# axoloto/CudaCam

Measured on AMD Instinct MI355X. Metric: frames/sec, 1920x1080 grayscale Canny (5-stage, Mode R, device-resident), higher is better.
Workload: dtype u8

## Files before the change

### cudacam_amd/api.py

```python
import ctypes as C
import enum
import os
import sys

import numpy as np

_HERE = os.path.dirname(os.path.abspath(__file__))
LIB_PATH = os.environ.get("HIPCANNY_LIB") or os.path.join(_HERE, "libhipcanny.so")


class CannyStage(enum.IntEnum):
    MONO = 0
    GAUSSIAN = 1
    GRADIENT = 2
    NMS = 3
    THRESH = 4
    HYSTER = 5


CANNY_STAGES = {
    CannyStage.MONO: "1/6 Mono Conversion",
    CannyStage.GAUSSIAN: "2/6 Gaussian Noise Removal",
    CannyStage.GRADIENT: "3/6 Gradient Computation",
    CannyStage.NMS: "4/6 Non Maximum Suppression",
# ... 4 lines not shown
MODE_R, MODE_O = 0, 1
OPT_NMS_SATURATE = 1
OPT_PIPELINE = 2
OPT_PER_CHANNEL = 3
OPT_FRONT_SPLIT = 4
OPT_L2_GRADIENT = 5
OPT_DEBUG_TAPS = 6
OPT_FRONT_HALF = 7
OPT_FRONT_DENSE = 8
OPT_COPY_STREAMS = 9
OPT_PIPELINE_SLOTS = 10
OPT_FRONT_WPB = 11
OPT_FRONT_MX = 12
OPT_APERTURE = 13
OPT_TEST_HYST_LATE_GRID, OPT_TEST_HYST_LOOP, OPT_TEST_HYST_DIAG, OPT_TEST_HYST_GEOM, OPT_TEST_DENSE_ENTER, OPT_TEST_DENSE_LEAVE = 100, 101, 102, 103, 104, 105
TAP_BLUR, TAP_THRESH = 1, 2
SCHEDULE_FIELDS = ("launches", "lists", "loop", "hist_grid", "longest", "overflows", "tiles", "tile_rows", "waves", "panels", "frames")

ABI_SYMBOLS = [
    "hc_create", "hc_destroy", "hc_set_thresholds", "hc_get_thresholds", "hc_upload", "hc_run", "hc_run_device",
    "hc_hysteresis_device", "hc_download", "hc_sync", "hc_set_stream", "hc_enable_profiling", "hc_stage_time_ms", "hc_profile_get",
    "hc_device_ptrs", "hc_last_hysteresis_info", "hc_hysteresis_stats", "hc_set_tuning", "hc_set_option", "hc_selftest", "hc_last_error", "hc_version",
    "hc_host_alloc", "hc_host_free", "hc_profile_get_front", "hc_debug_tap", "hc_use_own_stream", "hc_profile_get_intervals", "hc_last_run_info", "hc_pipeline_depth", "hc_pipeline_slots_in_use", "hc_front_waves_per_workgroup",
    "hc_profile_get_front_each", "hc_hysteresis_totals", "hc_last_hysteresis_schedule", "hc_download_begin", "hc_download_end", "hc_run_gradients_device",
]

_lib = None
_lib_legacy = None
LEGACY_LIB_PATH = os.path.join(_HERE, "libhipcanny_legacy.so")


class HipCannyError(RuntimeError):
    pass


def preload_hip_runtime():
    import importlib.util
    spec = importlib.util.find_spec("torch")
    if spec is None or not spec.origin:
# ... 40 lines not shown
    L.hc_device_ptrs.argtypes = [vp, C.POINTER(vp), C.POINTER(vp), C.POINTER(sz), C.POINTER(sz), C.POINTER(sz), C.POINTER(sz)]
    L.hc_last_hysteresis_info.argtypes = [vp, C.POINTER(i), C.POINTER(i)]
    L.hc_hysteresis_stats.argtypes = [vp, C.POINTER(C.c_uint), i]
    L.hc_set_tuning.argtypes = [vp, i, i]
    L.hc_set_option.argtypes = [vp, i, i]
    L.hc_selftest.argtypes = [i]
    L.hc_debug_tap.argtypes = [vp, i, vp, sz, sz, i]
    L.hc_last_run_info.argtypes = [vp, C.POINTER(i), C.POINTER(i), C.POINTER(i)]
    L.hc_pipeline_depth.argtypes = [vp, i]
    L.hc_pipeline_slots_in_use.argtypes = [vp]
    L.hc_front_waves_per_workgroup.argtypes = [vp]
    L.hc_profile_get_intervals.argtypes = [vp, C.POINTER(C.c_float), i, C.POINTER(i)]
    L.hc_profile_get_front_each.argtypes = [vp, C.POINTER(C.c_float), i, C.POINTER(i)]
    L.hc_hysteresis_totals.argtypes = [vp, C.POINTER(C.c_ulonglong), i]
    L.hc_last_hysteresis_schedule.argtypes = [vp, C.POINTER(i), i]
    L.hc_host_alloc.restype = vp
    L.hc_host_alloc.argtypes = [sz]
    L.hc_host_free.restype = None
    L.hc_host_free.argtypes = [vp]
    L.hc_last_error.restype = C.c_char_p
    L.hc_version.restype = C.c_char_p
    for name in ABI_SYMBOLS:
        getattr(L, name)
    if legacy:
        _lib_legacy = L
    else:
        _lib = L
    return L


# ... 81 lines not shown
    def profile_front_each(self, cap=4096):
        buf = (C.c_float * cap)()
        n = C.c_int()
        _ck(self.lib.hc_profile_get_front_each(self.handle, buf, cap, C.byref(n)))
        return [buf[k] for k in range(min(cap, n.value))]

    def hysteresis_totals(self, reset=False):
        t = (C.c_ulonglong * 4)()
        _ck(self.lib.hc_hysteresis_totals(self.handle, t, int(bool(reset))))
        return tuple(int(v) for v in t)

    def hysteresis_schedule(self):
        v = (C.c_int * len(SCHEDULE_FIELDS))()
        _ck(self.lib.hc_last_hysteresis_schedule(self.handle, v, len(SCHEDULE_FIELDS)))
        return dict(zip(SCHEDULE_FIELDS, (int(x) for x in v)))

    def profile_get_front(self):
        sums = (C.c_double * 2)()
        n = C.c_long()
        _ck(self.lib.hc_profile_get_front(self.handle, sums, C.byref(n)))
        return [sums[0], sums[1]], n.value

    def upload(self, frames):
        a = np.ascontiguousarray(frames, dtype=np.uint8)
        if a.ndim == (2 if self.c == 1 else 3):
            a = a[None]
        exp = (self.h, self.w) if self.c == 1 else (self.h, self.w, 3)
        if a.shape[1:] != exp:
            raise HipCannyError(f"Cannot load image to GPU, specs different since initialization: {a.shape[1:]} vs {exp}")
        row = self.w * self.c
# ... 237 lines not shown
```

### cudacam_amd/csrc/canny_common.h

```cpp
#pragma once
#include <hip/hip_runtime.h>
#include "canny_params.h"

namespace hc {

hipError_t launch_selftest(u32 *d_result, hipStream_t s);
hipError_t check_gauss_coeffs(const float gk[25]);
hipError_t launch_front_o(const FrontParams &p, hipStream_t s);
hipError_t launch_front_o_ext(const FrontExtParams &p, hipStream_t s);
#ifdef HC_LEGACY_FRONT
hipError_t launch_front(const FrontParams &p, hipStream_t s);
hipError_t launch_blur(const FrontParams &p, hipStream_t s);
hipError_t launch_nms(const FrontParams &p, hipStream_t s);
size_t front_lds_bytes();
#endif
hipError_t launch_front8(const FrontParams &p, hipStream_t s);
hipError_t launch_front8o(const FrontParams &p, hipStream_t s);
hipError_t launch_front_mx(const FrontParams &p, hipStream_t s);
hipError_t launch_hyst(const HystParams &p, hipStream_t s);
hipError_t launch_hyst_loop(const HystParams &p, int rounds, u32 *bar, hipStream_t s);
hipError_t launch_pack(const PackParams &p, hipStream_t s);
hipError_t launch_copy_rows(void *dst, size_t dpitch, size_t dfs, const void *src, size_t spitch, size_t sfs, size_t row_bytes, int rows, int n, hipStream_t s);

hipError_t launch_gray(const uint8_t *bgr, size_t bpitch, size_t bfs, uint8_t *mono, size_t mpitch, size_t mfs, int W, int H, int n, hipStream_t s);
hipError_t launch_gauss(const uint8_t *mono, size_t mpitch, size_t mfs, uint8_t *blur, size_t bpitch, size_t bfs, int W, int H, int n, hipStream_t s);
hipError_t launch_sobel(const uint8_t *blur, size_t bpitch, size_t bfs, int16_t *sx, int16_t *sy, size_t spitch_elems, size_t sfs_elems, int W, int H, int n, hipStream_t s);
hipError_t launch_graddisp(const int16_t *sx, const int16_t *sy, size_t spitch_elems, size_t sfs_elems, uint8_t *out, size_t opitch, size_t ofs, int W, int H, int n, hipStream_t s);
hipError_t launch_nms(const int16_t *sx, const int16_t *sy, size_t spitch_elems, size_t sfs_elems, uint8_t *out, size_t opitch, size_t ofs, int W, int H, int n, int saturate, hipStream_t s);
hipError_t launch_thresh(const uint8_t *nms, size_t npitch, size_t nfs, uint8_t *out, size_t opitch, size_t ofs, int W, int H, int n, int low, int high, hipStream_t s);

}
```

### cudacam_amd/csrc/canny_kernels.hip

```cpp
#include "canny_device.h"
#include <cstdio>
#include <cstdlib>
#include <cstring>
#include <type_traits>

namespace hc {

hipError_t check_gauss_coeffs(const float gk[25])
{
  return memcmp(gk, GKC.v, sizeof(GKC.v)) == 0 ? hipSuccess : hipErrorInvalidValue;
}

__global__ void k_selftest(u32 *res)
{
  const u32 lane = threadIdx.x & 63;
  u32 bad = 0;
  bad |= (from_lane_below(lane + 100) != (lane ? lane + 99 : 0)) ? 1u : 0u;
  bad |= (from_lane_above(lane + 100) != (lane < 63 ? lane + 101 : 0)) ? 2u : 0u;
  const u32 x = 0x44332211u + lane;
  bad |= (unpack_lo(x) != ((x & 0xFF) | (((x >> 8) & 0xFF) << 16))) ? 4u : 0u;
  bad |= (unpack_hi(x) != (((x >> 16) & 0xFF) | ((x >> 24) << 16))) ? 8u : 0u;
  bad |= (pair_shift(0xAAAA1111u + lane, 0x2222BBBBu) != (((0xAAAA1111u + lane) << 16) | 0x2222u)) ? 16u : 0u;
  const u32 p0 = 0x00050003u, p1 = 0x00090007u;
  bad |= (__builtin_amdgcn_perm(p1, p0, 0x06040200u) != 0x09070503u) ? 32u : 0u;
// ... 305 lines not shown
  uint8_t *d = dst + (size_t)f * dfs + (size_t)row * dpitch + x;
  if (x + 16u <= row_bytes) *reinterpret_cast<u32x4_any *>(d) = *reinterpret_cast<const u32x4_any *>(q);
  else
    for (unsigned k = 0; x + k < row_bytes; ++k) d[k] = q[k];
}

hipError_t launch_copy_rows(void *dst, size_t dpitch, size_t dfs, const void *src, size_t spitch, size_t sfs, size_t row_bytes, int rows, int n, hipStream_t s)
{
  if (row_bytes == 0 || rows <= 0 || n <= 0) return hipSuccess;
  if (row_bytes > 0x7FFFFFFFull || rows > 65535 || n > 65535) return hipErrorInvalidValue;
  const dim3 grid((unsigned)((row_bytes + 4095) / 4096), (unsigned)rows, (unsigned)n), block(256);
  hipLaunchKernelGGL(k_copy_rows, grid, block, 0, s, (uint8_t *)dst, dpitch, dfs, (const uint8_t *)src, spitch, sfs, (unsigned)row_bytes, rows);
  return hipGetLastError();
}

hipError_t launch_pack(const PackParams &p, hipStream_t s)
{
  const long long total = (long long)p.nframes * p.H * ((p.W + 255) / 256);
  hipLaunchKernelGGL(k_pack, dim3((unsigned)((total + 3) / 4)), dim3(256), 0, s, p);
  return hipGetLastError();
}

template <int NW>
struct RowBits {
  u32 w[NW];
};

template <int NW>
static __device__ __forceinline__ RowBits<NW> row_load(const u32 *plane_row, int lane, int RD)
{
// ... 691 lines not shown
```

### cudacam_amd/csrc/hipcanny.hip

```cpp
#include "../../include/hipcanny.h"
#include "canny_common.h"
#include "host_plan.h"

#include <algorithm>
#include <cstdio>
#include <cstdlib>
#include <cstring>
#include <mutex>
#include <string>
#include <vector>

using namespace hc;

namespace {
constexpr int MAX_DEVICES = 64;
hipStream_t g_h2d[MAX_DEVICES] = { nullptr }, g_d2h[MAX_DEVICES] = { nullptr };
std::mutex g_copy_streams_mutex;
thread_local std::string g_err;
int fail(int code, const std::string &msg)
{
  g_err = msg;
  return code;
}
#define HIPCK(expr)                                                                                   \
  do {                                                                                                \
    hipError_t e_ = (expr);                                                                           \
    if (e_ != hipSuccess) return fail(HC_E_HIP, std::string(#expr) + ": " + hipGetErrorString(e_));  \
  } while (0)

struct Slot {
  bool complete = false;
  u32 *d_sbits = nullptr, *d_cbits = nullptr;
  u32 *d_wl_list = nullptr;
  size_t wl_cap = 0;
  u32 *d_flags = nullptr, *h_flags = nullptr;
  hipEvent_t ev_front = nullptr, ev_done = nullptr;
  bool pending = false;
  HystParams ph{};
  HystPlan plan;
  void *copy_dst = nullptr;
  size_t copy_pitch = 0, copy_fs = 0;
  int n = 0;
  bool prov = false;
  hipStream_t stream = nullptr;
  hipStream_t s_hyst = nullptr;
  uintptr_t out0 = 0, out1 = 0;
  unsigned long long seq = 0;
};

struct ProfRing {
// ... 94 lines not shown
  size_t in_pitch = 0, in_fs = 0, mono_pitch = 0, mono_fs = 0, out_pitch = 0, out_fs = 0;
  uint8_t *d_blur = nullptr, *d_nms = nullptr;
  int16_t *d_sx = nullptr, *d_sy = nullptr;
  uint8_t *d_dump = nullptr;
  size_t dump_region = 0;
  uint8_t *d_bplane = nullptr;
  size_t bplane_fs = 0, bplane_frames = 0;
  Slot slot[NSLOT];
  int nslot_use = 2;
  int cur = 0;
  bool pipeline = false;
  unsigned long long run_seq = 0;
  ChainWatch watch;
  struct { hipEvent_t f[8] = {}, d[8] = {}; unsigned long long seq[8] = {}; } ring;
  HystHistory hist;
  ProfRing prof;
  struct {
    uint8_t *host = nullptr; size_t row = 0, fs = 0; int n = 0;
    bool stale = false;
  } dl;
  bool copy_streams = false;
  hipEvent_t ev_up = nullptr, ev_ready = nullptr, ev_ready2 = nullptr, ev_down = nullptr;
  struct {
    u32 *s = nullptr, *c = nullptr;
    uint8_t *blur = nullptr;
    int frames = 0;
    bool blur_split = false, blur_valid = false;
  } dbg;
  struct {
    int front_waves = 4;
// ... 29 lines not shown
  return HC_OK;
}

int alloc_slot_parts(hc_ctx *c, Slot &s)
{
  const size_t out_frames = (size_t)c->max_batch * (c->per_channel ? 3 : 1);
  const size_t plane_bytes = sizeof(u32) * (size_t)c->RD * c->H * out_frames;
  HIPCK(hipMalloc((void **)&s.d_sbits, plane_bytes));
  HIPCK(hipMalloc((void **)&s.d_cbits, plane_bytes));
  HIPCK(hipMemsetAsync(s.d_sbits, 0, plane_bytes, c->stream));
  HIPCK(hipMemsetAsync(s.d_cbits, 0, plane_bytes, c->stream));
  HIPCK(hipStreamSynchronize(c->stream));
  s.wl_cap = slot_wl_cap(out_frames, c->H, c->RD);
  HIPCK(hipMalloc((void **)&s.d_wl_list, sizeof(u32) * 2 * s.wl_cap));
  HIPCK(hipMalloc((void **)&s.d_flags, sizeof(u32) * run_flag_words(s.wl_cap)));
  HIPCK(hipHostMalloc((void **)&s.h_flags, sizeof(u32) * (FLAG_WORDS + WL_COUNT_WORDS), hipHostMallocDefault));
  {
    int least = 0, greatest = 0;
    (void)hipDeviceGetStreamPriorityRange(&least, &greatest);
    HIPCK(hipStreamCreateWithPriority(&s.s_hyst, hipStreamNonBlocking, greatest));
  }
  HIPCK(hipEventCreateWithFlags(&s.ev_front, hipEventDisableTiming));
  HIPCK(hipEventCreateWithFlags(&s.ev_done, hipEventDisableTiming));
  return HC_OK;
}

void free_slot(Slot &s)
{
  for (void *q : { (void *)s.d_sbits, (void *)s.d_cbits, (void *)s.d_wl_list, (void *)s.d_flags }) (void)hipFree(q);
  if (s.h_flags) (void)hipHostFree(s.h_flags);
  if (s.ev_front) (void)hipEventDestroy(s.ev_front);
// ... 1 lines not shown
  if (s.s_hyst) (void)hipStreamDestroy(s.s_hyst);
  s = Slot{};
}

int alloc_slot(hc_ctx *c, Slot &s)
{
  if (s.complete) return HC_OK;
  const int rc = alloc_slot_parts(c, s);
  if (rc != HC_OK) {
    const std::string why = g_err;
    free_slot(s);
    return fail(rc, why);
  }
  s.complete = true;
  return HC_OK;
}

#ifdef HC_LEGACY_FRONT
int ensure_blur_plane(hc_ctx *c)
{
  const size_t frames = (size_t)c->max_batch * (c->per_channel ? 3 : 1);
  if (c->d_bplane && c->bplane_frames == frames) return HC_OK;
  if (c->d_bplane) { (void)hipFree(c->d_bplane); c->d_bplane = nullptr; }
  c->bplane_fs = (size_t)c->nstrips * c->H * 256;
  HIPCK(hipMalloc((void **)&c->d_bplane, c->bplane_fs * frames));
  c->bplane_frames = frames;
  return HC_OK;
}
#endif

// ... 48 lines not shown
  if (c->ring.seq[b] != i || c->ring.seq[a] != i - 1 || i < 2) return;
  float front_ms = 0.0f, lead_ms = 0.0f;
  if (hipEventElapsedTime(&front_ms, c->ring.f[a], c->ring.f[b]) != hipSuccess || hipEventElapsedTime(&lead_ms, c->ring.d[a], c->ring.f[b]) != hipSuccess) {
    (void)hipGetLastError();
    return;
  }
  c->watch.update(i, c->nslot_use, front_ms, lead_ms);
}

int finish_slot(hc_ctx *c, Slot &s)
{
  if (!s.pending) return HC_OK;
  s.pending = false;
  s.out0 = s.out1 = 0;
  hipStream_t st = s.stream;
  HIPCK(hipEventSynchronize(s.ev_done));
  watch_chain(c, s);
  const HystPlan &p = s.plan;
  const int K = p.K;
  int work = 0;
  for (int k = 0; k < K; ++k) work += s.h_flags[k] != 0;
  work = std::min(K, work + 1);
  std::memcpy(c->last.stats, s.h_flags + MAX_HYST_LAUNCHES, sizeof(c->last.stats));
  c->last.continued = 0;
  c->last.totals[0] += 1;
  c->last.totals[3] += (unsigned long long)K;
  u32 wl_counts[MAX_HYST_LAUNCHES + 1];
  std::memcpy(wl_counts, s.h_flags + FLAG_WORDS, sizeof(wl_counts));
  {
    int *d = c->last.sched;
    d[HC_SCHED_LAUNCHES] = K; d[HC_SCHED_LISTS] = p.mixed ? 2 : p.lists0; d[HC_SCHED_LOOP] = p.loop ? 1 : 0;
// ... 3 lines not shown
      const u32 len = wl_counts[k];
      d[HC_SCHED_LONGEST] = std::max(d[HC_SCHED_LONGEST], (int)std::min<u32>(len, 0x7FFFFFFFu));
      if (p.hist_grid(k) <= 0) continue;
      d[HC_SCHED_HIST_GRID] = d[HC_SCHED_HIST_GRID] ? std::min(d[HC_SCHED_HIST_GRID], p.hist_grid(k)) : p.hist_grid(k);
      if (len > (u32)p.hist_grid(k)) d[HC_SCHED_OVERFLOWS] += 1;
    }
    d[HC_SCHED_TILES] = (int)std::min<size_t>(p.wl_stride, 0x7FFFFFFF); d[HC_SCHED_TILE_ROWS] = p.tile_rows; d[HC_SCHED_WAVES] = p.waves;
    d[HC_SCHED_PANELS] = p.npanels; d[HC_SCHED_FRAMES] = s.ph.nframes;
  }
  const bool converged = s.h_flags[K - 1] == 0;
  if (!converged) {
    c->last.continued = 1;
    c->last.totals[1] += 1;
    if (c->dl.host) c->dl.stale = true;
    for (int round = 0; round < 1000000; ++round) {
      HIPCK(hipMemsetAsync(s.d_flags, 0, sizeof(u32) * run_flag_words(p.wl_stride), st));
      HystParams hp = s.ph;
      hp.late_grid = p.test_grid;
      hp.first_pass = 0;
      hp.stats = nullptr;
      for (int k = 0; k < K; ++k) {
        hp.iter = k;
        hp.lists = p.lists[k];
        HIPCK(launch_hyst(hp, st));
      }
      HIPCK(hipMemcpyAsync(s.h_flags, s.d_flags, sizeof(u32) * (FLAG_WORDS + WL_COUNT_WORDS), hipMemcpyDeviceToHost, st));
      HIPCK(hipStreamSynchronize(st));
      for (int k = 0; k < K; ++k) work += s.h_flags[k] != 0;
      if (s.h_flags[K - 1] == 0) break;
    }
  }
  c->last.totals[2] += (unsigned long long)work;
  c->hist.finished(p, work, wl_counts);
  if (converged) return HC_OK;
  if (s.copy_dst)
    if (int rc = copy_frames_d2d(c, st, s.copy_dst, s.copy_pitch, s.copy_fs, s.ph.out, s.ph.out_pitch, s.ph.out_frame_stride, (size_t)c->W, s.n)) return rc;
  HIPCK(hipStreamSynchronize(st));
  return HC_OK;
}

int finish_all(hc_ctx *c)
// ... 15 lines not shown
  hp.tile_rows = p.tile_rows; hp.waves = p.waves; hp.nrtiles = p.nrtiles; hp.npanels = p.npanels;
  hp.out = out; hp.out_pitch = out_pitch; hp.out_frame_stride = out_fs; hp.W = c->W;
  hp.wl_stride = p.wl_stride;
  hp.wl_count = s.d_flags + FLAG_WORDS;
  hp.wl_reason = s.d_flags + FLAG_WORDS + WL_COUNT_WORDS;
  hp.wl_list = s.d_wl_list;
  hp.first_pass = 1;
  hp.prov = s.prov ? 1 : 0;
  if (p.clear) HIPCK(hipMemsetAsync(s.d_flags, 0, sizeof(u32) * run_flag_words(p.wl_stride), st));
  if (p.loop) HIPCK(launch_hyst_loop(hp, p.K, s.d_flags + FLAG_WORDS + WL_COUNT_WORDS - 2, st));
  for (int k = p.loop ? p.K : 0; k < p.K; ++k) {
    hp.iter = k; hp.lists = p.lists[k]; hp.late_grid = p.late_grid[k];
    hp.stats = c->hopt.diag ? s.d_flags + MAX_HYST_LAUNCHES + 3 * k : nullptr;
    HIPCK(launch_hyst(hp, st));
  }
  HIPCK(hipMemcpyAsync(s.h_flags, s.d_flags, sizeof(u32) * (FLAG_WORDS + WL_COUNT_WORDS), hipMemcpyDeviceToHost, st));
  s.pending = true;
  s.ph = hp;
  s.n = n;
  s.stream = st;
  s.copy_dst = nullptr;
  return HC_OK;
}

int rotate_slots(hc_ctx *c, bool piped, int n_out, Slot **slot)
{
  if (piped) {
    const int use = pipeline_slots(c->watch.pipe_slots, c->watch.big_slots, n_out, c->W, c->H);
    if (use != c->nslot_use) {
      if (int rc = finish_all(c)) return rc;
      c->nslot_use = use;
      c->cur = 0;
    }
  }
  Slot &s = c->slot[piped ? c->cur : 0];
  *slot = &s;
  if (!piped) { s.seq = 0; return finish_all(c); }
  if (int rc = alloc_slot(c, s)) return rc;
  if (int rc = finish_slot(c, s)) return rc;
  s.seq = ++c->run_seq;
  return HC_OK;
}

int finish_overlapping(hc_ctx *c, uintptr_t o0, uintptr_t o1, bool *with_previous)
{
  *with_previous = false;
  for (int k = 1; k < c->nslot_use; ++k) {
    Slot &o = c->slot[(c->cur + k) % c->nslot_use];
    if (!(o.out0 < o1 && o0 < o.out1)) continue;
    if (k == c->nslot_use - 1) *with_previous = true;
    if (int rc = finish_slot(c, o)) return rc;
  }
  return HC_OK;
}

int run_impl(hc_ctx *c, const uint8_t *in, size_t in_pitch, size_t in_fs, uint8_t *out, size_t out_pitch, size_t out_fs, int n, int stage,
// ... 3 lines not shown
    return fail(HC_E_ARG, "mode O (cv::Canny) produces the final edge map only (cv::Canny has no intermediate outputs)");
  if (c->mode == HC_MODE_O && c->per_channel) return fail(HC_E_ARG, "HC_OPT_PER_CHANNEL applies to mode R contexts");
  if (c->per_channel && stage != HC_STAGE_HYSTER) return fail(HC_E_ARG, "per-channel mode only produces the final edge maps (HC_STAGE_HYSTER)");
  const int W = c->W, H = c->H;
  const int n_out = c->per_channel ? 3 * n : n;
  const bool piped = c->pipeline && stage == HC_STAGE_HYSTER;
  Slot *slot = nullptr;
  if (int rc = rotate_slots(c, piped, n_out, &slot)) return rc;
  Slot &s = *slot;
  FrontIn fi{ c->mode, c->C, W, H, c->RD, c->nstrips, c->per_channel, stage, n };
  fi.in = View{ (uintptr_t)in, in_pitch, in_fs }; fi.out = View{ (uintptr_t)out, out_pitch, out_fs }; fi.in_dy = (uintptr_t)in_dy;
  fi.own_in = View{ 0, c->in_pitch, c->in_fs }; fi.own_mono = View{ 0, c->mono_pitch, c->mono_fs }; fi.own_out = View{ 0, c->out_pitch, c->out_fs };
  fi.o = c->opt; fi.dump_region = c->dump_region; fi.piped = piped; fi.nslot_use = c->nslot_use; fi.front_one = c->watch.front_one; fi.wl_cap = s.wl_cap;
  const bool out_internal = out_view_staged(fi.out);
  uint8_t *dst = out_internal ? c->d_out : out;
  if (piped) {
    const uintptr_t o0 = (uintptr_t)dst, o1 = o0 + (size_t)n_out * (out_internal ? c->out_fs : out_fs);
    if (int rc = finish_overlapping(c, o0, o1, &fi.out_overlap)) return rc;
    s.out0 = o0; s.out1 = o1;
  }
  const FrontPlan P = plan_front(fi);
  c->last.in_staged = P.in_staged ? 1 : 0;
  c->last.out_staged = P.out_staged ? 1 : 0;
  c->last.front_form = P.form;
  if (P.error) return fail(HC_E_ARG, P.error);
  hipStream_t sf = c->stream, sh = piped ? s.s_hyst : c->stream;
  const size_t dp = P.dst.pitch, dfs = P.dst.fs;
  const uint8_t *src = P.in_staged ? c->d_in : in;
  if (P.in_staged)
    if (int rc = copy_frames_d2d(c, sf, c->d_in, c->in_pitch, c->in_fs, in, in_pitch, in_fs, (size_t)W * c->C, n)) return rc;
  ProfRing &prof = c->prof;
  HIPCK(prof.begin_run(sf));
  const uint8_t *mono = src;
  if (P.gray) {
    uint8_t *grey = stage == HC_STAGE_MONO ? dst : c->d_mono;
    HIPCK(launch_gray(src, P.src.pitch, P.src.fs, grey, stage == HC_STAGE_MONO ? dp : c->mono_pitch, stage == HC_STAGE_MONO ? dfs : c->mono_fs, W, H, n, sf));
    if (stage != HC_STAGE_MONO) mono = c->d_mono;
    HIPCK(prof.mark(sf, B_MONO, ProfRing::K_STAGE0));
  } else if (stage == HC_STAGE_MONO) {
    if (int rc = copy_frames_d2d(c, sf, dst, dp, dfs, src, P.src.pitch, P.src.fs, (size_t)W, n)) return rc;
    HIPCK(prof.mark(sf, B_MONO, ProfRing::K_STAGE0));
  }
  const size_t mp = P.mono.pitch, mfs = P.mono.fs;

  if (stage == HC_STAGE_HYSTER) {
    FrontParams fp = P.fp;
    fp.in = mono; fp.sbits = s.d_sbits; fp.cbits = s.d_cbits;
    s.prov = P.prov;
    if (P.prov) fp.prov_out = dst;
    if (c->opt.debug_taps) {
      if (int rc = ensure_debug_buffers(c)) return rc;
      if (P.form != 1) fp.dbg_blur = c->dbg.blur;
    }
    if (P.zeroed_words) {
      const size_t R = c->dump_region;
      fp.zero_words = s.d_flags;
      fp.dump = c->d_dump; fp.dump_c = c->d_dump + (fp.half ? R : 2048); fp.dump_p = c->d_dump + (fp.half ? 2 * R : 4096);
      fp.zeros = c->d_dump + (fp.half ? 3 * R : 16384);
    }
    if (P.waves) c->last.front_waves = P.waves;
    switch (P.form) {
    case 6: case 7: {
      FrontExtParams ep{};
      ep.f = fp;
      ep.gradients = in_dy ? 1 : 0;
      ep.channels = c->C;
      ep.dy = in_dy;
      HIPCK(launch_front_o_ext(ep, sf));
      break;
    }
    case 3: HIPCK(launch_front8o(fp, sf)); break;
    case -1: HIPCK(launch_front_o(fp, sf)); break;
    case 5: HIPCK(launch_front_mx(fp, sf)); break;
    case 2: case 4: HIPCK(launch_front8(fp, sf)); break;
#ifdef HC_LEGACY_FRONT
    case 1:
      if (int rc = ensure_blur_plane(c)) return rc;
      fp.blur = c->d_bplane; fp.blur_frame_stride = c->bplane_fs;
      HIPCK(launch_blur(fp, sf));
      HIPCK(prof.mark(sf, P.mask_a, ProfRing::K_FRONT_A));
      HIPCK(launch_nms(fp, sf));
      break;
    case 0: HIPCK(launch_front(fp, sf)); break;
#endif
    default: return fail(HC_E_ARG, "internal: front kernel form");
    }
    HIPCK(prof.mark(sf, P.mask, ProfRing::K_FRONT_B));
    if (c->opt.debug_taps) {
      const size_t bytes = sizeof(u32) * (size_t)c->RD * H * (size_t)n_out;
      HIPCK(hipMemcpyAsync(c->dbg.s, s.d_sbits, bytes, hipMemcpyDeviceToDevice, sf));
      HIPCK(hipMemcpyAsync(c->dbg.c, s.d_cbits, bytes, hipMemcpyDeviceToDevice, sf));
      c->dbg.frames = n_out;
      c->dbg.blur_split = P.form == 1;
      c->dbg.blur_valid = c->mode == HC_MODE_R;
    }
    if (piped) {
      HIPCK(hipEventRecord(s.ev_front, sf));
      const int k = (int)(s.seq & 7);
      if (!c->ring.f[k]) { HIPCK(hipEventCreate(&c->ring.f[k])); HIPCK(hipEventCreate(&c->ring.d[k])); }
      HIPCK(hipEventRecord(c->ring.f[k], sf));
      c->ring.seq[k] = 0;
      HIPCK(hipStreamWaitEvent(sh, s.ev_front, 0));
    }
    if (int rc = queue_hyst_expand(c, s, sh, dst, dp, dfs, n_out, piped, P.zeroed_words)) return rc;
  } else if (stage > HC_STAGE_MONO) {
    if (int rc = ensure_stage_scratch(c)) return rc;
    const size_t bp = c->out_pitch, bfs = c->out_fs;
    uint8_t *blur = stage == HC_STAGE_GAUSSIAN ? dst : c->d_blur;
    const size_t blp = stage == HC_STAGE_GAUSSIAN ? dp : bp, blfs = stage == HC_STAGE_GAUSSIAN ? dfs : bfs;
    HIPCK(launch_gauss(mono, mp, mfs, blur, blp, blfs, W, H, n, sf));
    HIPCK(prof.mark(sf, B_GAUSS, ProfRing::K_FRONT_B));
    if (stage >= HC_STAGE_GRADIENT) {
      HIPCK(launch_sobel(blur, blp, blfs, c->d_sx, c->d_sy, bp, bfs, W, H, n, sf));
      if (stage == HC_STAGE_GRADIENT) HIPCK(launch_graddisp(c->d_sx, c->d_sy, bp, bfs, dst, dp, dfs, W, H, n, sf));
      HIPCK(prof.mark(sf, B_GRAD, ProfRing::K_FRONT_B));
      if (stage > HC_STAGE_GRADIENT) {
        uint8_t *nms = stage == HC_STAGE_NMS ? dst : c->d_nms;
        const size_t np = stage == HC_STAGE_NMS ? dp : bp, nfs = stage == HC_STAGE_NMS ? dfs : bfs;
// ... 4 lines not shown
          HIPCK(prof.mark(sf, B_THR, ProfRing::K_FRONT_B));
        }
      }
    }
  }

  if (out_internal) {
    if (int rc = copy_frames_d2d(c, sh, out, out_pitch, out_fs, c->d_out, c->out_pitch, c->out_fs, (size_t)W, n_out)) return rc;
    if (s.pending) { s.copy_dst = out; s.copy_pitch = out_pitch; s.copy_fs = out_fs; }
  }
  if (stage == HC_STAGE_HYSTER) HIPCK(prof.mark(sh, B_HYST, ProfRing::K_HYST));
  else if (out_internal) HIPCK(prof.mark(sh, 1u << stage, ProfRing::K_FRONT_B));
  prof.end_run();
  if (stage == HC_STAGE_HYSTER) HIPCK(hipEventRecord(s.ev_done, sh));
  if (piped) {
    HIPCK(hipEventRecord(c->ring.d[s.seq & 7], sh));
    c->ring.seq[s.seq & 7] = s.seq;
  }
  c->last.slot = piped ? c->cur : 0;
  if (piped) c->cur = (c->cur + 1) % c->nslot_use;
  c->last.run_n = n_out;
  return HC_OK;
}

}

extern "C" {

const char *hc_last_error(void) { return g_err.c_str(); }
#ifdef HC_LEGACY_FRONT
const char *hc_version(void) { return "hipcanny 0.4 (gfx950) + round-1 front kernels (test build)"; }
#else
// ... 54 lines not shown
    volatile float r = 1 / 159.0f;
    for (int i = 0; i < 25; ++i) { volatile float k = (float)K[i]; volatile float v = k * r; gk[i] = v; }
    good = ok(check_gauss_coeffs(gk), "Gaussian coefficient table differs from the kernels' literals");
  }
  if (!good) { hc_destroy(c); return nullptr; }
  return c;
}

void hc_destroy(hc_ctx *c)
{
  if (!c) return;
  (void)hipSetDevice(c->device);
  (void)hipDeviceSynchronize();
  for (void *q : { (void *)c->d_in, (void *)c->d_mono, (void *)c->d_out, (void *)c->d_blur, (void *)c->d_nms, (void *)c->d_sx, (void *)c->d_sy, (void *)c->d_bplane, (void *)c->d_dump }) (void)hipFree(q);
  for (Slot &q : c->slot) free_slot(q);
  free_debug_buffers(c);
  for (auto &e : c->prof.evpool) if (e) (void)hipEventDestroy(e);
  for (hipEvent_t e : { c->ev_up, c->ev_ready, c->ev_ready2, c->ev_down }) if (e) (void)hipEventDestroy(e);
  for (hipEvent_t e : c->ring.f) if (e) (void)hipEventDestroy(e);
  for (hipEvent_t e : c->ring.d) if (e) (void)hipEventDestroy(e);
  if (c->own_stream) (void)hipStreamDestroy(c->own_stream);
  delete c;
}

int hc_set_thresholds(hc_ctx *c, int low, int high)
{
  if (!c) return fail(HC_E_ARG, "null context");
  const int tmax = c->mode == HC_MODE_O ? 32767 : 255;
  low = std::max(0, std::min(tmax, low));
  high = std::max(0, std::min(tmax, high));
// ... 36 lines not shown
  c->hopt.launches_set = hyst_launches != 0;
  c->hopt.launches = hyst_launches ? hyst_launches : 6;
  return HC_OK;
}

int hc_set_option(hc_ctx *c, int option, int value)
{
  if (!c) return fail(HC_E_ARG, "null context");
  if (int rc = finish_all(c)) return rc;
  if (option == HC_OPT_NMS_SATURATE) c->opt.nms_saturate = value != 0;
  else if (option == HC_OPT_PER_CHANNEL) {
    if (c->C != 3) return fail(HC_E_ARG, "HC_OPT_PER_CHANNEL needs a 3-channel context");
    if ((value != 0) != (c->per_channel != 0)) {
      HIPCK(hipSetDevice(c->device));
      HIPCK(hipDeviceSynchronize());
      for (Slot &q : c->slot) free_slot(q);
      (void)hipFree(c->d_out);
      c->d_out = nullptr;
      c->per_channel = value != 0;
      free_debug_buffers(c);
      if (c->d_bplane) { (void)hipFree(c->d_bplane); c->d_bplane = nullptr; c->bplane_frames = 0; }
      if (alloc_frames(&c->d_out, &c->out_pitch, &c->out_fs, (size_t)c->W, c->H, c->max_batch * (c->per_channel ? 3 : 1), (size_t)c->W) != HC_OK) return HC_E_HIP;
      if (alloc_slot(c, c->slot[0]) != HC_OK) return HC_E_HIP;
    }
  } else if (option == HC_OPT_FRONT_SPLIT) {
    if (value < 0 || value > 2) return fail(HC_E_ARG, "HC_OPT_FRONT_SPLIT: 0 (k_front), 1 (k_blur + k_nms) or 2 (k_front8)");
#ifndef HC_LEGACY_FRONT
    if (value != 2 && c->mode == HC_MODE_R)
      return fail(HC_E_ARG, "HC_OPT_FRONT_SPLIT 1 / 0: the round-1 front kernels are not part of this library (parity tests load libhipcanny_legacy.so)");
#endif
// ... 20 lines not shown
    else return fail(HC_E_ARG, "HC_OPT_PIPELINE_SLOTS: -1 (automatic), 2, 3, or 20 / 21 (diagnostics)");
  } else if (option == HC_OPT_FRONT_DENSE) {
    if (value < -1 || value > 1) return fail(HC_E_ARG, "HC_OPT_FRONT_DENSE: -1 (automatic), 0 (never) or 1 (every window)");
    c->opt.dense_mode = value;
  } else if (option == HC_OPT_FRONT_MX) {
    if (value != 0 && value != 1) return fail(HC_E_ARG, "HC_OPT_FRONT_MX: 0 (never) or 1 (whenever the run allows it)");
    c->opt.mx_mode = value;
  } else if (option == HC_OPT_TEST_HYST_LATE_GRID) {
    c->hopt.late_grid = std::max(-1, value);
  } else if (option == HC_OPT_TEST_HYST_LOOP) {
    c->hopt.loop = value != 0;
  } else if (option == HC_OPT_TEST_HYST_DIAG) {
    c->hopt.diag = value != 0;
  } else if (option == HC_OPT_TEST_HYST_GEOM) {
    c->hopt.geom = std::max(0, value);
  } else if (option == HC_OPT_TEST_DENSE_ENTER) {
    c->opt.dense_enter = std::max(0, value);
  } else if (option == HC_OPT_TEST_DENSE_LEAVE) {
    c->opt.dense_leave = std::max(0, value);
  } else if (option == HC_OPT_FRONT_HALF) {
    if (value < -1 || value > 1) return fail(HC_E_ARG, "HC_OPT_FRONT_HALF: -1 (automatic), 0 (never) or 1 (whenever possible)");
    HIPCK(hipSetDevice(c->device));
    if (value == 1 && !c->dump_region) {
      HIPCK(hipDeviceSynchronize());
      if (int rc = alloc_dump(c, true)) return rc;
    }
    c->opt.half_mode = value;
  } else if (option == HC_OPT_L2_GRADIENT) {
    if (c->mode != HC_MODE_O) return fail(HC_E_ARG, "HC_OPT_L2_GRADIENT applies to mode O contexts");
    c->opt.l2gradient = value != 0;
// ... 340 lines not shown
  if (!c || !info) return fail(HC_E_ARG, "null argument");
  if (int rc = finish_all(c)) return rc;
  for (int i = 0; i < nwords && i < HC_SCHED_WORDS; ++i) info[i] = c->last.sched[i];
  return HC_OK;
}

int hc_hysteresis_totals(hc_ctx *c, unsigned long long totals[4], int reset)
{
  if (!c || !totals) return fail(HC_E_ARG, "null argument");
  if (int rc = finish_all(c)) return rc;
  for (int i = 0; i < 4; ++i) totals[i] = c->last.totals[i];
  if (reset) for (int i = 0; i < 4; ++i) c->last.totals[i] = 0;
  return HC_OK;
}

int hc_selftest(int device)
{
  int ndev = 0;
  if (hipGetDeviceCount(&ndev) != hipSuccess || device < 0 || device >= ndev) return fail(HC_E_NOGPU, "hc_selftest: no HIP device");
  HIPCK(hipSetDevice(device));
  u32 *d = nullptr, h = 0xFFFFFFFFu;
  HIPCK(hipMalloc((void **)&d, sizeof(u32)));
  HIPCK(hipMemset(d, 0, sizeof(u32)));
  HIPCK(launch_selftest(d, nullptr));
  HIPCK(hipMemcpy(&h, d, sizeof(u32), hipMemcpyDeviceToHost));
  (void)hipFree(d);
  if (h) return fail(HC_E_HIP, "hc_selftest: primitive check failed, bits=" + std::to_string(h));
  return HC_OK;
}
}
// ... 1 lines not shown
```

### cudacam_amd/csrc/host_plan.h

```cpp
#pragma once
#include "../../include/hipcanny.h"
#include "canny_params.h"

#include <algorithm>

namespace hc {

inline size_t round_up(size_t v, size_t a) { return (v + a - 1) / a * a; }
inline bool aligned4(uintptr_t p, size_t a, size_t b) { return ((p | a | b) & 3u) == 0; }
inline bool reaches_4g(int H, size_t pitch) { return (unsigned long long)H * pitch >= (1ull << 32); }

constexpr int MAX_HYST_LAUNCHES = 96;
constexpr int FLAG_WORDS = MAX_HYST_LAUNCHES * 4;
constexpr int WL_COUNT_WORDS = 128;
static_assert(WL_COUNT_WORDS >= MAX_HYST_LAUNCHES + 1 + 2, "a count per launch, one beyond the last, and the two words of k_hyst_loop's barrier");
inline size_t slot_wl_cap(size_t out_frames, int H, int RD) { return out_frames * ((size_t)(H + 15) / 16 + 1) * (size_t)((RD + 63) / 64); }
inline size_t run_flag_words(size_t wl_stride) { return FLAG_WORDS + WL_COUNT_WORDS + 2 * wl_stride; }

inline size_t frame_pitch(size_t row_bytes, size_t tight_row_bytes) { return (tight_row_bytes && tight_row_bytes % 16 == 0) ? tight_row_bytes : round_up(row_bytes, 256); }
inline int plane_row_dwords(int W)
{
  const size_t need = std::max<size_t>((size_t)(W + 31) / 32, ((size_t)((W + STRIP_W - 1) / STRIP_W) * 31 + 3) / 4);
  return need > 256 ? 0 : need <= 64 ? 64 : need <= 128 ? 128 : 256;
}
inline bool half_pays(int W) { return front8_half_strips(W) % 2 == 1 || (front8_half_strips(W) + 1) / 2 < front8_strips(W); }
inline size_t half_dump_region(size_t in_fs, size_t out_fs, int RD, int H) { return round_up(std::max(std::max(in_fs, 3 * out_fs), 3 * sizeof(u32) * (size_t)RD * H) + 32768, 4096); }

constexpr int NSLOT = 4;
inline int pipeline_slots(int pipe_slots, int big_slots, int n_out, int W, int H) { return pipe_slots ? pipe_slots : (long long)n_out * H * W < 500ll * 1000 * 1000 ? NSLOT : big_slots; }
inline int pipeline_depth(bool pipeline, int pipe_slots, int big_slots, int n_out, int W, int H)
{
  if (!pipeline) return 1;
  const int n = pipeline_slots(pipe_slots, big_slots, n_out, W, H);
  return (n < NSLOT && !pipe_slots) ? 3 : n;
}

struct ChainWatch {
  int pipe_slots = 0;
  int chain_told = 0;
  int big_slots = 2;
  bool front_one = false;
  float slack_ema = 0.0f;
  int chain_bound_runs = 0, chain_light_runs = 0, chain_light_needed = 16;
  float period_ms[4] = { 0, 0, 0, 0 }, period_two = 0.0f;
  int trial_runs = -1;
  int retry_wait = 0, retry_backoff = 64;

  void update(unsigned long long i, int nslot_use, float front_ms, float lead_ms)
  {
// ... 360 lines not shown
```

### include/hipcanny.h

```cpp
#ifndef HIPCANNY_H
#define HIPCANNY_H

#include <stddef.h>
#include <stdint.h>

#ifdef __cplusplus
extern "C" {
#endif

typedef struct hc_ctx hc_ctx;

enum { HC_STAGE_MONO = 0, HC_STAGE_GAUSSIAN = 1, HC_STAGE_GRADIENT = 2, HC_STAGE_NMS = 3, HC_STAGE_THRESH = 4, HC_STAGE_HYSTER = 5 };

enum { HC_MODE_R = 0, HC_MODE_O = 1 };

enum {
  HC_OK = 0,
  HC_E_ARG = -1,
  HC_E_HIP = -2,
  HC_E_STATE = -3,
  HC_E_NOGPU = -4
};

hc_ctx *hc_create(int device, int width, int height, int channels, int max_batch, int mode);
// ... 47 lines not shown
int hc_last_hysteresis_schedule(hc_ctx *ctx, int *info, int nwords);

int hc_last_run_info(hc_ctx *ctx, int *input_staged, int *output_staged, int *front_form);

int hc_pipeline_depth(hc_ctx *ctx, int nframes);
int hc_pipeline_slots_in_use(hc_ctx *ctx);
int hc_front_waves_per_workgroup(hc_ctx *ctx);

int hc_hysteresis_stats(hc_ctx *ctx, unsigned *stats, int nwords);

int hc_set_tuning(hc_ctx *ctx, int chunk_rows, int hyst_launches);

enum { HC_OPT_NMS_SATURATE = 1, HC_OPT_PIPELINE = 2, HC_OPT_PER_CHANNEL = 3, HC_OPT_FRONT_SPLIT = 4, HC_OPT_L2_GRADIENT = 5, HC_OPT_DEBUG_TAPS = 6, HC_OPT_FRONT_HALF = 7,
       HC_OPT_FRONT_DENSE = 8, HC_OPT_COPY_STREAMS = 9, HC_OPT_PIPELINE_SLOTS = 10, HC_OPT_FRONT_WPB = 11, HC_OPT_FRONT_MX = 12, HC_OPT_APERTURE = 13,
       HC_OPT_TEST_HYST_LATE_GRID = 100, HC_OPT_TEST_HYST_LOOP = 101, HC_OPT_TEST_HYST_DIAG = 102, HC_OPT_TEST_HYST_GEOM = 103,
       HC_OPT_TEST_DENSE_ENTER = 104, HC_OPT_TEST_DENSE_LEAVE = 105 };
int hc_set_option(hc_ctx *ctx, int option, int value);

enum { HC_TAP_BLUR = 1, HC_TAP_THRESH = 2 };
int hc_debug_tap(hc_ctx *ctx, int what, uint8_t *host, size_t row_stride, size_t frame_stride, int nframes);

void *hc_host_alloc(size_t bytes);
void hc_host_free(void *p);

int hc_selftest(int device);

const char *hc_last_error(void);
const char *hc_version(void);

#ifdef __cplusplus
}
#endif
// ... 2 lines not shown
```

Measured before the change: 305,100.

## Queue next front kernel before finishing busy slot using spare bit planes

When a pipeline slot is still busy, the host now enqueues the next frame's front kernel into spare sbits/cbits/flags buffers first, and only then blocks on finishing the previous hysteresis. This keeps the GPU fed instead of stalling the host on the event sync. The device-to-host flag copy is also replaced by a tiny kernel writing into mapped coherent host memory. The change adds an extra set of buffers, buffer swapping logic and trace instrumentation, and risks ordering bugs with the swapped planes.

```diff
diff --git a/cudacam_amd/api.py b/cudacam_amd/api.py
--- a/cudacam_amd/api.py
+++ b/cudacam_amd/api.py
@@ -42,6 +42,9 @@
 OPT_FRONT_MX = 12
 OPT_APERTURE = 13
 OPT_TEST_HYST_LATE_GRID, OPT_TEST_HYST_LOOP, OPT_TEST_HYST_DIAG, OPT_TEST_HYST_GEOM, OPT_TEST_DENSE_ENTER, OPT_TEST_DENSE_LEAVE = 100, 101, 102, 103, 104, 105
+OPT_TEST_QUEUE_TRACE, OPT_TEST_QUEUE_ORDER = 106, 107
+TEST_QUEUE_TRACE, TEST_FLAG_WORDS, QT_WORDS = 1, 2, 8
+QT_FIELDS = ("run", "front_first", "slot_done", "front_call_us", "front_called_us", "wait_in_us", "wait_out_us", "chain_us")
 TAP_BLUR, TAP_THRESH = 1, 2
 SCHEDULE_FIELDS = ("launches", "lists", "loop", "hist_grid", "longest", "overflows", "tiles", "tile_rows", "waves", "panels", "frames")
 
@@ -51,6 +54,7 @@
     "hc_device_ptrs", "hc_last_hysteresis_info", "hc_hysteresis_stats", "hc_set_tuning", "hc_set_option", "hc_selftest", "hc_last_error", "hc_version",
     "hc_host_alloc", "hc_host_free", "hc_profile_get_front", "hc_debug_tap", "hc_use_own_stream", "hc_profile_get_intervals", "hc_last_run_info", "hc_pipeline_depth", "hc_pipeline_slots_in_use", "hc_front_waves_per_workgroup",
     "hc_profile_get_front_each", "hc_hysteresis_totals", "hc_last_hysteresis_schedule", "hc_download_begin", "hc_download_end", "hc_run_gradients_device",
+    "hc_test_read",
 ]
 
 _lib = None
@@ -121,6 +125,7 @@
     L.hc_profile_get_front_each.argtypes = [vp, C.POINTER(C.c_float), i, C.POINTER(i)]
     L.hc_hysteresis_totals.argtypes = [vp, C.POINTER(C.c_ulonglong), i]
     L.hc_last_hysteresis_schedule.argtypes = [vp, C.POINTER(i), i]
+    L.hc_test_read.argtypes = [vp, i, vp, i, C.POINTER(i)]
     L.hc_host_alloc.restype = vp
     L.hc_host_alloc.argtypes = [sz]
     L.hc_host_free.restype = None
@@ -232,6 +237,20 @@
         v = (C.c_int * len(SCHEDULE_FIELDS))()
         _ck(self.lib.hc_last_hysteresis_schedule(self.handle, v, len(SCHEDULE_FIELDS)))
         return dict(zip(SCHEDULE_FIELDS, (int(x) for x in v)))
+
+    def queue_trace(self):
+        n = C.c_int()
+        _ck(self.lib.hc_test_read(self.handle, TEST_QUEUE_TRACE, None, 0, C.byref(n)))
+        buf = (C.c_double * (n.value // 8))()
+        _ck(self.lib.hc_test_read(self.handle, TEST_QUEUE_TRACE, buf, n.value, C.byref(n)))
+        return [dict(zip(QT_FIELDS, buf[k:k + QT_WORDS])) for k in range(0, len(buf), QT_WORDS)]
+
+    def flag_words(self):
+        n = C.c_int()
+        _ck(self.lib.hc_test_read(self.handle, TEST_FLAG_WORDS, None, 0, C.byref(n)))
+        buf = np.zeros(n.value // 4, np.uint32)
+        _ck(self.lib.hc_test_read(self.handle, TEST_FLAG_WORDS, buf.ctypes.data, n.value, C.byref(n)))
+        return buf[:len(buf) // 2].copy(), buf[len(buf) // 2:].copy()
 
     def profile_get_front(self):
         sums = (C.c_double * 2)()
diff --git a/cudacam_amd/csrc/canny_common.h b/cudacam_amd/csrc/canny_common.h
--- a/cudacam_amd/csrc/canny_common.h
+++ b/cudacam_amd/csrc/canny_common.h
@@ -21,6 +21,7 @@
 hipError_t launch_hyst_loop(const HystParams &p, int rounds, u32 *bar, hipStream_t s);
 hipError_t launch_pack(const PackParams &p, hipStream_t s);
 hipError_t launch_copy_rows(void *dst, size_t dpitch, size_t dfs, const void *src, size_t spitch, size_t sfs, size_t row_bytes, int rows, int n, hipStream_t s);
+hipError_t launch_flags_out(u32 *dst_mapped, const u32 *d_src, int nwords, hipStream_t s);
 
 hipError_t launch_gray(const uint8_t *bgr, size_t bpitch, size_t bfs, uint8_t *mono, size_t mpitch, size_t mfs, int W, int H, int n, hipStream_t s);
 hipError_t launch_gauss(const uint8_t *mono, size_t mpitch, size_t mfs, uint8_t *blur, size_t bpitch, size_t bfs, int W, int H, int n, hipStream_t s);
diff --git a/cudacam_amd/csrc/canny_kernels.hip b/cudacam_amd/csrc/canny_kernels.hip
--- a/cudacam_amd/csrc/canny_kernels.hip
+++ b/cudacam_amd/csrc/canny_kernels.hip
@@ -343,6 +343,19 @@
   return hipGetLastError();
 }
 
+__global__ __launch_bounds__(64) void k_flags_out(u32 *dst, const u32 *src, int nwords)
+{
+  for (int i = (int)threadIdx.x; i < nwords; i += 64) dst[i] = src[i];
+  __threadfence_system();
+}
+
+hipError_t launch_flags_out(u32 *dst_mapped, const u32 *d_src, int nwords, hipStream_t s)
+{
+  if (!dst_mapped || !d_src || nwords <= 0) return hipErrorInvalidValue;
+  hipLaunchKernelGGL(k_flags_out, dim3(1), dim3(64), 0, s, dst_mapped, d_src, nwords);
+  return hipGetLastError();
+}
+
 hipError_t launch_pack(const PackParams &p, hipStream_t s)
 {
   const long long total = (long long)p.nframes * p.H * ((p.W + 255) / 256);
diff --git a/cudacam_amd/csrc/hipcanny.hip b/cudacam_amd/csrc/hipcanny.hip
--- a/cudacam_amd/csrc/hipcanny.hip
+++ b/cudacam_amd/csrc/hipcanny.hip
@@ -3,6 +3,7 @@
 #include "host_plan.h"
 
 #include <algorithm>
+#include <chrono>
 #include <cstdio>
 #include <cstdlib>
 #include <cstring>
@@ -34,6 +35,7 @@
   u32 *d_wl_list = nullptr;
   size_t wl_cap = 0;
   u32 *d_flags = nullptr, *h_flags = nullptr;
+  u32 *h_flags_dev = nullptr;
   hipEvent_t ev_front = nullptr, ev_done = nullptr;
   bool pending = false;
   HystParams ph{};
@@ -158,6 +160,15 @@
   ChainWatch watch;
   struct { hipEvent_t f[8] = {}, d[8] = {}; unsigned long long seq[8] = {}; } ring;
   HystHistory hist;
+  struct { u32 *sbits = nullptr, *cbits = nullptr, *flags = nullptr; bool busy = false; } spare;
+  bool finish_first = false;
+  struct {
+    bool on = false;
+    std::chrono::steady_clock::time_point t0;
+    double wait_in = 0, wait_out = 0;
+    std::vector<double> rec;
+    double now() const { return std::chrono::duration<double, std::micro>(std::chrono::steady_clock::now() - t0).count(); }
+  } qt;
   ProfRing prof;
   struct {
     uint8_t *host = nullptr; size_t row = 0, fs = 0; int n = 0;
@@ -217,7 +228,8 @@
   s.wl_cap = slot_wl_cap(out_frames, c->H, c->RD);
   HIPCK(hipMalloc((void **)&s.d_wl_list, sizeof(u32) * 2 * s.wl_cap));
   HIPCK(hipMalloc((void **)&s.d_flags, sizeof(u32) * run_flag_words(s.wl_cap)));
-  HIPCK(hipHostMalloc((void **)&s.h_flags, sizeof(u32) * (FLAG_WORDS + WL_COUNT_WORDS), hipHostMallocDefault));
+  HIPCK(hipHostMalloc((void **)&s.h_flags, sizeof(u32) * (FLAG_WORDS + WL_COUNT_WORDS), hipHostMallocMapped | hipHostMallocCoherent));
+  HIPCK(hipHostGetDevicePointer((void **)&s.h_flags_dev, s.h_flags, 0));
   {
     int least = 0, greatest = 0;
     (void)hipDeviceGetStreamPriorityRange(&least, &greatest);
@@ -249,6 +261,34 @@
   }
   s.complete = true;
   return HC_OK;
+}
+
+int ensure_spare(hc_ctx *c)
+{
+  if (c->spare.flags) return HC_OK;
+  const size_t out_frames = (size_t)c->max_batch * (c->per_channel ? 3 : 1);
+  const size_t plane_bytes = sizeof(u32) * (size_t)c->RD * c->H * out_frames;
+  u32 *sb = nullptr, *cb = nullptr, *fl = nullptr;
+  hipError_t e = hipMalloc((void **)&sb, plane_bytes);
+  if (e == hipSuccess) e = hipMalloc((void **)&cb, plane_bytes);
+  if (e == hipSuccess) e = hipMalloc((void **)&fl, sizeof(u32) * run_flag_words(slot_wl_cap(out_frames, c->H, c->RD)));
+  if (e == hipSuccess) e = hipMemsetAsync(sb, 0, plane_bytes, c->stream);
+  if (e == hipSuccess) e = hipMemsetAsync(cb, 0, plane_bytes, c->stream);
+  if (e == hipSuccess) e = hipStreamSynchronize(c->stream);
+  if (e != hipSuccess) {
+    for (void *q : { (void *)sb, (void *)cb, (void *)fl }) (void)hipFree(q);
+    (void)hipGetLastError();
+    return fail(HC_E_HIP, std::string("spare plane set: ") + hipGetErrorString(e));
+  }
+  c->spare.sbits = sb; c->spare.cbits = cb; c->spare.flags = fl;
+  return HC_OK;
+}
+
+void free_spare(hc_ctx *c)
+{
+  for (void *q : { (void *)c->spare.sbits, (void *)c->spare.cbits, (void *)c->spare.flags }) (void)hipFree(q);
+  c->spare.sbits = c->spare.cbits = c->spare.flags = nullptr;
+  c->spare.busy = false;
 }
 
 #ifdef HC_LEGACY_FRONT
@@ -327,7 +367,9 @@
   s.pending = false;
   s.out0 = s.out1 = 0;
   hipStream_t st = s.stream;
+  if (c->qt.on) c->qt.wait_in = c->qt.now();
   HIPCK(hipEventSynchronize(s.ev_done));
+  if (c->qt.on) c->qt.wait_out = c->qt.now();
   watch_chain(c, s);
   const HystPlan &p = s.plan;
   const int K = p.K;
@@ -361,7 +403,7 @@
     c->last.totals[1] += 1;
     if (c->dl.host) c->dl.stale = true;
     for (int round = 0; round < 1000000; ++round) {
-      HIPCK(hipMemsetAsync(s.d_flags, 0, sizeof(u32) * run_flag_words(p.wl_stride), st));
+      HIPCK(hipMemsetAsync(s.ph.flags, 0, sizeof(u32) * run_flag_words(p.wl_stride), st));
       HystParams hp = s.ph;
       hp.late_grid = p.test_grid;
       hp.first_pass = 0;
@@ -371,7 +413,7 @@
         hp.lists = p.lists[k];
         HIPCK(launch_hyst(hp, st));
       }
-      HIPCK(hipMemcpyAsync(s.h_flags, s.d_flags, sizeof(u32) * (FLAG_WORDS + WL_COUNT_WORDS), hipMemcpyDeviceToHost, st));
+      HIPCK(launch_flags_out(s.h_flags_dev, s.ph.flags, FLAG_WORDS + WL_COUNT_WORDS, st));
       HIPCK(hipStreamSynchronize(st));
       for (int k = 0; k < K; ++k) work += s.h_flags[k] != 0;
       if (s.h_flags[K - 1] == 0) break;
@@ -417,7 +459,7 @@
     hp.stats = c->hopt.diag ? s.d_flags + MAX_HYST_LAUNCHES + 3 * k : nullptr;
     HIPCK(launch_hyst(hp, st));
   }
-  HIPCK(hipMemcpyAsync(s.h_flags, s.d_flags, sizeof(u32) * (FLAG_WORDS + WL_COUNT_WORDS), hipMemcpyDeviceToHost, st));
+  HIPCK(launch_flags_out(s.h_flags_dev, s.d_flags, FLAG_WORDS + WL_COUNT_WORDS, st));
   s.pending = true;
   s.ph = hp;
   s.n = n;
@@ -439,10 +481,7 @@
   Slot &s = c->slot[piped ? c->cur : 0];
   *slot = &s;
   if (!piped) { s.seq = 0; return finish_all(c); }
-  if (int rc = alloc_slot(c, s)) return rc;
-  if (int rc = finish_slot(c, s)) return rc;
-  s.seq = ++c->run_seq;
-  return HC_OK;
+  return alloc_slot(c, s);
 }
 
 int finish_overlapping(hc_ctx *c, uintptr_t o0, uintptr_t o1, bool *with_previous)
@@ -476,11 +515,27 @@
   fi.o = c->opt; fi.dump_region = c->dump_region; fi.piped = piped; fi.nslot_use = c->nslot_use; fi.front_one = c->watch.front_one; fi.wl_cap = s.wl_cap;
   const bool out_internal = out_view_staged(fi.out);
   uint8_t *dst = out_internal ? c->d_out : out;
+  const uintptr_t o0 = (uintptr_t)dst, o1 = o0 + (size_t)n_out * (out_internal ? c->out_fs : out_fs);
+  bool front_first = false;
+  double qrec[HC_QT_WORDS] = { 0 };
   if (piped) {
-    const uintptr_t o0 = (uintptr_t)dst, o1 = o0 + (size_t)n_out * (out_internal ? c->out_fs : out_fs);
-    if (int rc = finish_overlapping(c, o0, o1, &fi.out_overlap)) return rc;
-    s.out0 = o0; s.out1 = o1;
-  }
+    bool done = true, overlap = false;
+    if (s.pending) {
+      done = hipEventQuery(s.ev_done) == hipSuccess;
+      if (!done) (void)hipGetLastError();
+      for (const Slot &q : c->slot) overlap = overlap || (q.pending && ranges_overlap(q.out0, q.out1, o0, o1));
+    }
+    front_first = queue_front_first(piped, s.pending, done, overlap, c->spare.busy, c->finish_first);
+    if (front_first && ensure_spare(c) != HC_OK) front_first = false;
+    qrec[1] = front_first ? 1 : 0; qrec[2] = s.pending ? (done ? 1 : 0) : -1;
+    c->qt.wait_in = c->qt.wait_out = 0;
+    if (!front_first) {
+      if (int rc = finish_slot(c, s)) return rc;
+      if (int rc = finish_overlapping(c, o0, o1, &fi.out_overlap)) return rc;
+    }
+  }
+  const unsigned long long seq = piped ? ++c->run_seq : 0;
+  if (!front_first) { s.seq = seq; if (piped) { s.out0 = o0; s.out1 = o1; } }
   const FrontPlan P = plan_front(fi);
   c->last.in_staged = P.in_staged ? 1 : 0;
   c->last.out_staged = P.out_staged ? 1 : 0;
@@ -506,9 +561,12 @@
   const size_t mp = P.mono.pitch, mfs = P.mono.fs;
 
   if (stage == HC_STAGE_HYSTER) {
+    if (front_first) {
+      std::swap(s.d_sbits, c->spare.sbits); std::swap(s.d_cbits, c->spare.cbits); std::swap(s.d_flags, c->spare.flags);
+      c->spare.busy = true;
+    }
     FrontParams fp = P.fp;
     fp.in = mono; fp.sbits = s.d_sbits; fp.cbits = s.d_cbits;
-    s.prov = P.prov;
     if (P.prov) fp.prov_out = dst;
     if (c->opt.debug_taps) {
       if (int rc = ensure_debug_buffers(c)) return rc;
@@ -521,6 +579,7 @@
       fp.zeros = c->d_dump + (fp.half ? 3 * R : 16384);
     }
     if (P.waves) c->last.front_waves = P.waves;
+    if (c->qt.on) qrec[3] = c->qt.now();
     switch (P.form) {
     case 6: case 7: {
       FrontExtParams ep{};
@@ -547,6 +606,7 @@
 #endif
     default: return fail(HC_E_ARG, "internal: front kernel form");
     }
+    if (c->qt.on) qrec[4] = c->qt.now();
     HIPCK(prof.mark(sf, P.mask, ProfRing::K_FRONT_B));
     if (c->opt.debug_taps) {
       const size_t bytes = sizeof(u32) * (size_t)c->RD * H * (size_t)n_out;
@@ -558,12 +618,25 @@
     }
     if (piped) {
       HIPCK(hipEventRecord(s.ev_front, sf));
-      const int k = (int)(s.seq & 7);
+      const int k = (int)(seq & 7);
       if (!c->ring.f[k]) { HIPCK(hipEventCreate(&c->ring.f[k])); HIPCK(hipEventCreate(&c->ring.d[k])); }
       HIPCK(hipEventRecord(c->ring.f[k], sf));
       c->ring.seq[k] = 0;
+    }
+    if (front_first) {
+      const int rc = finish_slot(c, s);
+      c->spare.busy = false;
+      if (rc) return rc;
+      s.seq = seq; s.out0 = o0; s.out1 = o1;
+    }
+    if (piped) {
       HIPCK(hipStreamWaitEvent(sh, s.ev_front, 0));
-    }
+      if (c->qt.on && c->qt.rec.size() < (size_t)HC_QT_WORDS * 4096) {
+        qrec[0] = (double)seq; qrec[5] = c->qt.wait_in; qrec[6] = c->qt.wait_out; qrec[7] = c->qt.now();
+        c->qt.rec.insert(c->qt.rec.end(), qrec, qrec + HC_QT_WORDS);
+      }
+    }
+    s.prov = P.prov;
     if (int rc = queue_hyst_expand(c, s, sh, dst, dp, dfs, n_out, piped, P.zeroed_words)) return rc;
   } else if (stage > HC_STAGE_MONO) {
     if (int rc = ensure_stage_scratch(c)) return rc;
@@ -598,8 +671,8 @@
   prof.end_run();
   if (stage == HC_STAGE_HYSTER) HIPCK(hipEventRecord(s.ev_done, sh));
   if (piped) {
-    HIPCK(hipEventRecord(c->ring.d[s.seq & 7], sh));
-    c->ring.seq[s.seq & 7] = s.seq;
+    HIPCK(hipEventRecord(c->ring.d[seq & 7], sh));
+    c->ring.seq[seq & 7] = seq;
   }
   c->last.slot = piped ? c->cur : 0;
   if (piped) c->cur = (c->cur + 1) % c->nslot_use;
@@ -684,6 +757,7 @@
   (void)hipDeviceSynchronize();
   for (void *q : { (void *)c->d_in, (void *)c->d_mono, (void *)c->d_out, (void *)c->d_blur, (void *)c->d_nms, (void *)c->d_sx, (void *)c->d_sy, (void *)c->d_bplane, (void *)c->d_dump }) (void)hipFree(q);
   for (Slot &q : c->slot) free_slot(q);
+  free_spare(c);
   free_debug_buffers(c);
   for (auto &e : c->prof.evpool) if (e) (void)hipEventDestroy(e);
   for (hipEvent_t e : { c->ev_up, c->ev_ready, c->ev_ready2, c->ev_down }) if (e) (void)hipEventDestroy(e);
@@ -750,6 +824,7 @@
     if ((value != 0) != (c->per_channel != 0)) {
       HIPCK(hipSetDevice(c->device));
       HIPCK(hipDeviceSynchronize());
+      free_spare(c);
       for (Slot &q : c->slot) free_slot(q);
       (void)hipFree(c->d_out);
       c->d_out = nullptr;
@@ -800,6 +875,11 @@
     c->hopt.diag = value != 0;
   } else if (option == HC_OPT_TEST_HYST_GEOM) {
     c->hopt.geom = std::max(0, value);
+  } else if (option == HC_OPT_TEST_QUEUE_TRACE) {
+    c->qt.on = value != 0;
+    if (c->qt.on) { c->qt.rec.clear(); c->qt.t0 = std::chrono::steady_clock::now(); }
+  } else if (option == HC_OPT_TEST_QUEUE_ORDER) {
+    c->finish_first = value == 0;
   } else if (option == HC_OPT_TEST_DENSE_ENTER) {
     c->opt.dense_enter = std::max(0, value);
   } else if (option == HC_OPT_TEST_DENSE_LEAVE) {
@@ -1170,6 +1250,30 @@
   return HC_OK;
 }
 
+int hc_test_read(hc_ctx *c, int what, void *out, int cap_bytes, int *nbytes)
+{
+  if (!c || !nbytes || cap_bytes < 0 || (cap_bytes > 0 && !out)) return fail(HC_E_ARG, "hc_test_read: bad argument");
+  HIPCK(hipSetDevice(c->device));
+  if (int rc = hc_sync(c)) return rc;
+  if (what == HC_TEST_QUEUE_TRACE) {
+    const size_t have = c->qt.rec.size() * sizeof(double);
+    std::memcpy(out, c->qt.rec.data(), std::min(have, (size_t)cap_bytes));
+    *nbytes = (int)have;
+    return HC_OK;
+  }
+  if (what == HC_TEST_FLAG_WORDS) {
+    const Slot &s = c->slot[c->last.slot];
+    const size_t half = sizeof(u32) * (FLAG_WORDS + WL_COUNT_WORDS);
+    if (!s.ph.flags) return fail(HC_E_STATE, "hc_test_read: no HC_STAGE_HYSTER run yet");
+    *nbytes = (int)(2 * half);
+    if ((size_t)cap_bytes < 2 * half) return HC_OK;
+    std::memcpy(out, s.h_flags, half);
+    HIPCK(hipMemcpy((uint8_t *)out + half, s.ph.flags, half, hipMemcpyDeviceToHost));
+    return HC_OK;
+  }
+  return fail(HC_E_ARG, "hc_test_read: unknown item");
+}
+
 int hc_selftest(int device)
 {
   int ndev = 0;
diff --git a/cudacam_amd/csrc/host_plan.h b/cudacam_amd/csrc/host_plan.h
--- a/cudacam_amd/csrc/host_plan.h
+++ b/cudacam_amd/csrc/host_plan.h
@@ -33,6 +33,12 @@
   if (!pipeline) return 1;
   const int n = pipeline_slots(pipe_slots, big_slots, n_out, W, H);
   return (n < NSLOT && !pipe_slots) ? 3 : n;
+}
+
+inline bool ranges_overlap(uintptr_t a0, uintptr_t a1, uintptr_t b0, uintptr_t b1) { return a0 < b1 && b0 < a1; }
+inline bool queue_front_first(bool piped, bool slot_pending, bool slot_done, bool out_overlaps_in_flight, bool spare_busy, bool finish_first)
+{
+  return piped && slot_pending && !slot_done && !out_overlaps_in_flight && !spare_busy && !finish_first;
 }
 
 struct ChainWatch {
diff --git a/include/hipcanny.h b/include/hipcanny.h
--- a/include/hipcanny.h
+++ b/include/hipcanny.h
@@ -85,8 +85,12 @@
 enum { HC_OPT_NMS_SATURATE = 1, HC_OPT_PIPELINE = 2, HC_OPT_PER_CHANNEL = 3, HC_OPT_FRONT_SPLIT = 4, HC_OPT_L2_GRADIENT = 5, HC_OPT_DEBUG_TAPS = 6, HC_OPT_FRONT_HALF = 7,
        HC_OPT_FRONT_DENSE = 8, HC_OPT_COPY_STREAMS = 9, HC_OPT_PIPELINE_SLOTS = 10, HC_OPT_FRONT_WPB = 11, HC_OPT_FRONT_MX = 12, HC_OPT_APERTURE = 13,
        HC_OPT_TEST_HYST_LATE_GRID = 100, HC_OPT_TEST_HYST_LOOP = 101, HC_OPT_TEST_HYST_DIAG = 102, HC_OPT_TEST_HYST_GEOM = 103,
-       HC_OPT_TEST_DENSE_ENTER = 104, HC_OPT_TEST_DENSE_LEAVE = 105 };
+       HC_OPT_TEST_DENSE_ENTER = 104, HC_OPT_TEST_DENSE_LEAVE = 105,
+       HC_OPT_TEST_QUEUE_TRACE = 106, HC_OPT_TEST_QUEUE_ORDER = 107 };
 int hc_set_option(hc_ctx *ctx, int option, int value);
+
+enum { HC_TEST_QUEUE_TRACE = 1, HC_TEST_FLAG_WORDS = 2, HC_QT_WORDS = 8 };
+int hc_test_read(hc_ctx *ctx, int what, void *out, int cap_bytes, int *nbytes);
 
 enum { HC_TAP_BLUR = 1, HC_TAP_THRESH = 2 };
 int hc_debug_tap(hc_ctx *ctx, int what, uint8_t *host, size_t row_stride, size_t frame_stride, int nframes);
```

Measured after the change: 305,000 (median of 2 runs). No clear change (-0.0%).
